# yurimjeon1892/EFGH

Measured on AMD Instinct MI355X. Metric: frame-pairs/sec EFGHNet fwd+bwd (384x1280 RGB + 64x2048 range), whole job, higher is better.
Workload: dtype f32; 1 GPU; BASELINE.json configs[2]: EFGHNet fwd+bwd with efghloss + gradient all-reduce + fused Adam, synthetic 384x1280 RGB + 131072-point sweep, batch=8 per GPU, random-init weights; global_batch=8, points=131072, parallelism=dp1

## Files before the change

### efgh_amd/csrc/wgrad.hip

```cpp
#include "common.h"

namespace {

typedef float f32x16 __attribute__((ext_vector_type(16)));
constexpr int TK = 128, TM = 32, LD = 128;

struct WArgs {
    const float *A; int64_t lda;
    int C, T, K;
    unsigned magicC;
    int Hin, Win, Hv, Wv, sh, sw;
    unsigned long long dhpack, dwpack;
    int Ho, Wo, osh, osw, oh0, ow0;
    const int *table;
    const float *G; int64_t ldg;
    int N;
    int tld;
    long long M; int mchunk;
    float *dW;
    long long zstride;
    unsigned kt, nt;
    long long bsA, bsG, bsD;
};

// ... 64 lines not shown
    }
    float4 rg[NGQ], ra[4];
    auto load_step = [&](long long ms) {
        if (TN != 128) {
#pragma unroll
            for (int q = 0; q < NGQ; ++q) {
                long long m = ms + gr0 + GRS * q;
                float4 g = make_float4(0.f, 0.f, 0.f, 0.f);
                if (m < mend && nin) g = *reinterpret_cast<const float4 *>(MODE == 1 ? git[q].g : p.G + m * p.ldg + n0 + gc4);
                rg[q] = g;
                if (MODE == 1) advance(git[q], n0 + gc4);
            }
        }
#pragma unroll
        for (int q = 0; q < 4; ++q) {
            long long m = ms + r0 + 8 * q;
            float4 g = make_float4(0.f, 0.f, 0.f, 0.f), a = g;
            if (m < mend) {
                if (MODE == 1) {
                    if (TN == 128 && nin) g = *reinterpret_cast<const float4 *>(rit[q].g);
                    if (kin && rit[q].rowok && (unsigned)(rit[q].j * p.sw + dw) < (unsigned)p.Win)
                        a = *reinterpret_cast<const float4 *>(rit[q].a);
                } else {
                    long long arow = -1;
                    if (MODE == 0) arow = m;
                    else if (kin) arow = p.table[m * (MODE == 4 ? p.tld : 16) + t];
                    if (TN == 128 && nin) g = *reinterpret_cast<const float4 *>(p.G + m * p.ldg + n0 + c4);
                    if (kin && arow >= 0) a = *reinterpret_cast<const float4 *>(p.A + arow * p.lda + c);
                }
            }
            if (TN == 128) rg[q] = g;
            ra[q] = a;
            if (MODE == 1) advance(rit[q], n0 + c4);
        }
    };

    f32x16 acc[2][TJ];
#pragma unroll
    for (int i = 0; i < 2; ++i)
#pragma unroll
        for (int j = 0; j < TJ; ++j)
#pragma unroll
            for (int r = 0; r < 16; ++r) acc[i][j][r] = 0.f;

    load_step(mbeg);
    for (long long ms = mbeg; ms < mend; ms += TM) {
#pragma unroll
        for (int q = 0; q < 4; ++q)
            *reinterpret_cast<float4 *>(&As[(r0 + 8 * q) * LD + c4]) = ra[q];
#pragma unroll
        for (int q = 0; q < NGQ; ++q)
            *reinterpret_cast<float4 *>(&Gs[(gr0 + GRS * q) * TN + gc4]) = rg[q];
        __syncthreads();
        if (ms + TM < mend) load_step(ms + TM);
#pragma unroll
        for (int mm = 0; mm < TM / 2; ++mm) {
            float g[2], a[TJ];
#pragma unroll
            for (int i = 0; i < 2; ++i) g[i] = Gs[(mm * 2 + lh) * TN + (wn * 2 + i) * 32 + l31];
#pragma unroll
            for (int j = 0; j < TJ; ++j) a[j] = As[(mm * 2 + lh) * LD + (wk * TJ + j) * 32 + l31];
#pragma unroll
            for (int i = 0; i < 2; ++i)
#pragma unroll
                for (int j = 0; j < TJ; ++j)
                    acc[i][j] = __builtin_amdgcn_mfma_f32_32x32x2f32(g[i], a[j], acc[i][j], 0, 0, 0);
        }
        __syncthreads();
    }
#pragma unroll
    for (int i = 0; i < 2; ++i)
#pragma unroll
        for (int j = 0; j < TJ; ++j) {
            const int k = k0 + (wk * TJ + j) * 32 + l31;
            if (k >= p.K) continue;
#pragma unroll
            for (int r = 0; r < 16; ++r) {
                const int n = n0 + (wn * 2 + i) * 32 + (r & 3) + 8 * (r >> 2) + 4 * lh;
                if (n < p.N) p.dW[(long long)n * p.K + k] = acc[i][j][r];
            }
        }
}

typedef efgh_wgrad_out_desc FoldUnpackArgs;

template <bool UNPACK>
__global__ void __launch_bounds__(256) k_fold_splits(const float4 *part, int zs, long long total4, float4 *dst, const FoldUnpackArgs u) {
    __shared__ float4 red[256];
    const int e = threadIdx.x & 15, zl = threadIdx.x >> 4;
    const long long i = (long long)blockIdx.x * 16 + e;
    float4 a = make_float4(0.f, 0.f, 0.f, 0.f), b = a;
    if (i < total4) {
        int z = zl;
        for (; z + 16 < zs; z += 32) {
            const float4 u = part[(long long)z * total4 + i], v = part[(long long)(z + 16) * total4 + i];
            a.x += u.x; a.y += u.y; a.z += u.z; a.w += u.w;
            b.x += v.x; b.y += v.y; b.z += v.z; b.w += v.w;
        }
        if (z < zs) { const float4 u = part[(long long)z * total4 + i]; a.x += u.x; a.y += u.y; a.z += u.z; a.w += u.w; }
        a.x += b.x; a.y += b.y; a.z += b.z; a.w += b.w;
    }
    red[threadIdx.x] = a;
    __syncthreads();
    for (int h = 8; h; h >>= 1) {
        if (zl < h) {
            const float4 o = red[threadIdx.x + h * 16];
            float4 m = red[threadIdx.x];
            m.x += o.x; m.y += o.y; m.z += o.z; m.w += o.w;
            red[threadIdx.x] = m;
        }
        __syncthreads();
    }
    if (zl == 0 && i < total4) {
        if (!UNPACK) { dst[i] = red[e]; return; }
        const float4 v4 = red[e];
        const float v[4] = {v4.x, v4.y, v4.z, v4.w};
        const long long idx = 4 * i;
        const int c0 = (int)(idx % u.Cp); const long long r = idx / u.Cp;
        const int t = (int)(r % u.T), n = (int)(r / u.T);
        if (n >= u.N) return;
        int ti = 0;
#pragma unroll
        for (int q = 0; q < 16; ++q) if (q == t) ti = u.taps[q];
#pragma unroll
        for (int q = 0; q < 4; ++q) {
            if (c0 + q >= u.C) continue;
            float *d = &u.W[n * u.sn + (c0 + q) * u.sc + ti * u.st];
            *d = u.accumulate ? *d + v[q] : v[q];
        }
    }
}

__global__ void k_unpack_weight(const float *__restrict__ Wp, float *__restrict__ W, int N, int T, int C,
                                int Cp, long long sn, long long sc, long long st, const int4 taps0,
                                const int4 taps1, const int4 taps2, const int4 taps3, int accumulate) {
    const int tp[16] = {taps0.x, taps0.y, taps0.z, taps0.w, taps1.x, taps1.y, taps1.z, taps1.w,
                        taps2.x, taps2.y, taps2.z, taps2.w, taps3.x, taps3.y, taps3.z, taps3.w};
    long long total = (long long)N * T * C;
    for (long long i = (long long)blockIdx.x * blockDim.x + threadIdx.x; i < total;
         i += (long long)gridDim.x * blockDim.x) {
        int c = (int)(i % C); long long r = i / C;
        int t = (int)(r % T); int n = (int)(r / T);
        int ti = 0;
#pragma unroll
        for (int q = 0; q < 16; ++q) if (q == t) ti = tp[q];
        float v = Wp[((long long)n * T + t) * Cp + c];
        float *dst = &W[n * sn + c * sc + ti * st];
        *dst = accumulate ? *dst + v : v;
    }
}

__global__ void __launch_bounds__(256)
k_table_scatter_add(const float *__restrict__ src, const int *__restrict__ table, long long M, int T, int C,
                    float *__restrict__ dst) {
    const int c4n = C >> 2;
    long long total = M * T * c4n;
    for (long long i = (long long)blockIdx.x * 256 + threadIdx.x; i < total; i += (long long)gridDim.x * 256) {
        int cq = (int)(i % c4n); long long r = i / c4n;
        int t = (int)(r % T); long long m = r / T;
        int row = table[m * 16 + t];
        if (row < 0) continue;
        float4 v = *reinterpret_cast<const float4 *>(src + (m * T + t) * C + cq * 4);
        float *d = dst + (long long)row * C + cq * 4;
        atomicAdd(d + 0, v.x); atomicAdd(d + 1, v.y); atomicAdd(d + 2, v.z); atomicAdd(d + 3, v.w);
    }
}

}

bool efgh_launch_fold_splits(const float *part, int zs, long long total, float *dst, hipStream_t st, const efgh_wgrad_out_desc *out) {
    const long long total4 = total / 4;
    const unsigned grid = (unsigned)((total4 + 15) / 16);
    if (out && out->W && out->T >= 1 && out->T <= 16 && out->Cp >= out->C && out->Cp % 4 == 0) {
        const long long row = (long long)out->T * out->Cp;
        if (total % row == 0 && total / row >= out->N && total / row < out->N + 4) {
            k_fold_splits<true><<<grid, 256, 0, st>>>((const float4 *)part, zs, total4, (float4 *)dst, *out);
            return true;
        }
    }
    FoldUnpackArgs none = {};
    k_fold_splits<false><<<grid, 256, 0, st>>>((const float4 *)part, zs, total4, (float4 *)dst, none);
    return false;
}

static int gather_wgrad_impl(const efgh_gemm_desc *d, const float *G, int64_t ldg, float *dWp, float *workspace, int nbatch,
                             int64_t bsG, int64_t bsD, const efgh_wgrad_out_desc *out, void *stream_, int tld = 0);


static long long wgrad_chunks(const efgh_gemm_desc *d, int nbatch, long long *chunk_out) {
    const int K = d->T * d->C;
    const int TN = d->N <= 64 ? 64 : 128;
    const long long kt = (K + TK - 1) / TK, nt = (d->N + TN - 1) / TN;
    static const int occ128[3] = {efgh_wg_per_cu((const void *)k_gather_wgrad<0, 128>, 256, 0), efgh_wg_per_cu((const void *)k_gather_wgrad<1, 128>, 256, 0),
                                  efgh_wg_per_cu((const void *)k_gather_wgrad<2, 128>, 256, 0)};
    static const int occ64[3] = {efgh_wg_per_cu((const void *)k_gather_wgrad<0, 64>, 256, 0), efgh_wg_per_cu((const void *)k_gather_wgrad<1, 64>, 256, 0),
                                 efgh_wg_per_cu((const void *)k_gather_wgrad<2, 64>, 256, 0)};
    const int mode = d->mode >= 0 && d->mode <= 2 ? d->mode : 0;
    return efgh_round_chunks(d->M, kt * nt * nbatch, TN == 128 ? occ128[mode] : occ64[mode], TM, 256, (double)nbatch * d->N * K, chunk_out);
}

extern "C" int64_t efgh_gather_wgrad_workspace(const efgh_gemm_desc *d) {
    if (!d || d->C <= 0 || d->T < 1 || d->N < 1 || d->M < 1) return 0;
    const int nbatch = d->nbatch > 1 ? d->nbatch : 1;
    const long long zs = wgrad_chunks(d, nbatch, nullptr);
    return zs > 1 ? zs * nbatch * (int64_t)d->N * d->T * d->C : 0;
}

extern "C" int efgh_gather_wgrad(const efgh_gemm_desc *d, const float *G, int64_t ldg, float *dWp, float *workspace,
                                 const efgh_wgrad_out_desc *out, void *stream_) {
    return gather_wgrad_impl(d, G, ldg, dWp, workspace, 1, 0, 0, out, stream_);
}

extern "C" int efgh_gather_wgrad_batched(const efgh_gemm_desc *d, const float *G, int64_t ldg, int64_t batch_stride_g,
                                         float *dWp, int64_t batch_stride_dw, float *workspace, void *stream_) {
    EFGH_CHECK_ARG(d && d->mode == 0 && d->nbatch >= 1 && d->nbatch <= 65535);
    EFGH_CHECK_ARG(d->batch_stride_a % 4 == 0 && batch_stride_g % 4 == 0 && batch_stride_dw == (int64_t)d->N * d->C);
    return gather_wgrad_impl(d, G, ldg, dWp, workspace, d->nbatch, batch_stride_g, batch_stride_dw, nullptr, stream_);
}

static int gather_wgrad_impl(const efgh_gemm_desc *d, const float *G, int64_t ldg, float *dWp, float *workspace, int nbatch,
                             int64_t bsG, int64_t bsD, const efgh_wgrad_out_desc *out, void *stream_, int tld) {
    hipStream_t st = (hipStream_t)stream_;
    EFGH_CHECK_ARG(d && d->A && G && dWp);
    EFGH_CHECK_ARG(d->C > 0 && d->C % 4 == 0 && d->T >= 1 && (d->T <= 16 || tld > 0) && d->N >= 1 && d->M >= 1);
    EFGH_CHECK_ARG(tld == 0 || (d->mode == 2 && d->table != nullptr && tld >= d->T && nbatch == 1 && !out));
    EFGH_CHECK_ARG(d->lda % 4 == 0 && ldg % 4 == 0 && d->N % 4 == 0);
    EFGH_CHECK_ARG((((uintptr_t)d->A) & 15) == 0 && (((uintptr_t)G) & 15) == 0 && (((uintptr_t)dWp) & 15) == 0);
    EFGH_CHECK_ARG((int64_t)d->T * d->C < 65536 && d->mode >= 0 && d->mode <= 2);
    WArgs a;
    a.A = d->A; a.lda = d->lda; a.C = d->C; a.T = d->T; a.K = d->T * d->C;
    a.magicC = (unsigned)((0x100000000ULL + d->C - 1) / d->C);
    a.Hin = d->Hin; a.Win = d->Win; a.Hv = d->Hv; a.Wv = d->Wv; a.sh = d->sh; a.sw = d->sw;
    a.dhpack = 0; a.dwpack = 0;
    for (int t = 0; t < 16; ++t) {
        int dh = t < d->T ? d->dh[t] : 0, dw = t < d->T ? d->dw[t] : 0;
        a.dhpack |= (unsigned long long)((dh + 8) & 15) << (4 * t);
        a.dwpack |= (unsigned long long)((dw + 8) & 15) << (4 * t);
    }
    a.Ho = d->Ho; a.Wo = d->Wo; a.osh = d->osh; a.osw = d->osw; a.oh0 = d->oh0; a.ow0 = d->ow0;
    a.table = d->table; a.G = G; a.ldg = ldg; a.N = d->N; a.M = d->M;
    a.bsA = nbatch > 1 ? d->batch_stride_a : 0; a.bsG = bsG; a.bsD = bsD; a.tld = tld;
    if (d->mode == 1) EFGH_CHECK_ARG(d->M == (int64_t)d->B * d->Hv * d->Wv && d->osh >= 1 && d->osw >= 1);
    if (d->mode == 2) EFGH_CHECK_ARG(d->table != nullptr);
    const int TN = a.N <= 64 ? 64 : 128;
    const int kt = (a.K + TK - 1) / TK, nt = (a.N + TN - 1) / TN;
    long long chunk = 0;
    const long long zs = wgrad_chunks(d, nbatch, &chunk);
    a.mchunk = (int)chunk;
    EFGH_CHECK_ARG(zs * kt * nt < 0x7fffffffLL);
    a.kt = (unsigned)kt; a.nt = (unsigned)nt;
    const long long plane = (long long)nbatch * a.N * a.K;
    EFGH_CHECK_ARG(zs == 1 || (workspace && (((uintptr_t)workspace) & 15) == 0));
    a.dW = zs > 1 ? workspace : dWp;
    a.zstride = zs > 1 ? plane : 0;
    const dim3 grid((unsigned)(zs * kt * nt), (unsigned)nbatch);
    if (tld > 0) {
        if (TN == 128) k_gather_wgrad<4, 128><<<grid, 256, 0, st>>>(a);
        else k_gather_wgrad<4, 64><<<grid, 256, 0, st>>>(a);
    } else if (TN == 128) {
        if (d->mode == 0) k_gather_wgrad<0, 128><<<grid, 256, 0, st>>>(a);
        else if (d->mode == 1) k_gather_wgrad<1, 128><<<grid, 256, 0, st>>>(a);
        else k_gather_wgrad<2, 128><<<grid, 256, 0, st>>>(a);
    } else {
        if (d->mode == 0) k_gather_wgrad<0, 64><<<grid, 256, 0, st>>>(a);
        else if (d->mode == 1) k_gather_wgrad<1, 64><<<grid, 256, 0, st>>>(a);
        else k_gather_wgrad<2, 64><<<grid, 256, 0, st>>>(a);
    }
    bool wrote = false;
    if (zs > 1) wrote = efgh_launch_fold_splits(workspace, (int)zs, plane, dWp, st, nbatch == 1 ? out : nullptr);
    EFGH_CHECK_LAUNCH();
    return wrote ? EFGH_WROTE_OUT : EFGH_OK;
}

extern "C" int efgh_blur_r_wgrad(const efgh_gemm_desc *d, int32_t ld, const float *G, int64_t ldg, float *dWp, float *workspace,
                                 void *stream_) {
    EFGH_CHECK_ARG(ld > 0);
    const int rc = gather_wgrad_impl(d, G, ldg, dWp, workspace, 1, 0, 0, nullptr, stream_, ld);
    return rc == EFGH_WROTE_OUT ? EFGH_OK : rc;
}

extern "C" int efgh_unpack_weight(const float *Wp, float *W, int32_t N, int32_t T, int32_t C, int32_t Cp,
                                  int64_t sn, int64_t sc, int64_t stt, const int32_t *tapidx, int32_t accumulate,
                                  void *stream_) {
    EFGH_CHECK_ARG(Wp && W && N > 0 && T > 0 && T <= 16 && C > 0 && Cp >= C);
    int tp[16];
    for (int t = 0; t < 16; ++t) tp[t] = (tapidx && t < T) ? tapidx[t] : (t < T ? t : 0);
    long long total = (long long)N * T * C;
    int grid = (int)((total + 255) / 256);
    if (grid > 8192) grid = 8192;
    k_unpack_weight<<<grid, 256, 0, (hipStream_t)stream_>>>(Wp, W, N, T, C, Cp, sn, sc, stt,
                                                           make_int4(tp[0], tp[1], tp[2], tp[3]),
                                                           make_int4(tp[4], tp[5], tp[6], tp[7]),
                                                           make_int4(tp[8], tp[9], tp[10], tp[11]),
                                                           make_int4(tp[12], tp[13], tp[14], tp[15]), accumulate);
    EFGH_CHECK_LAUNCH();
    return EFGH_OK;
}

extern "C" int efgh_table_scatter_add(const float *src, const int32_t *table, int64_t M, int32_t T, int32_t C,
                                      float *dst, void *stream_) {
    EFGH_CHECK_ARG(src && table && dst && M > 0 && T > 0 && T <= 16 && C % 4 == 0);
    long long total = M * T * (C / 4);
    long long g = (total + 255) / 256;
    k_table_scatter_add<<<(int)(g > 16384 ? 16384 : g), 256, 0, (hipStream_t)stream_>>>(src, table, M, T, C, dst);
    EFGH_CHECK_LAUNCH();
    return EFGH_OK;
}

extern "C" int efgh_debug_occupancy(char *out, int32_t cap) {
    EFGH_CHECK_ARG(out && cap > 64);
    snprintf(out, cap, "k_gather_wgrad<0,128> %d  <1,128> %d  <2,128> %d  <0,64> %d  <1,64> %d  <2,64> %d workgroups per CU",
             efgh_wg_per_cu((const void *)k_gather_wgrad<0, 128>, 256, 0), efgh_wg_per_cu((const void *)k_gather_wgrad<1, 128>, 256, 0),
             efgh_wg_per_cu((const void *)k_gather_wgrad<2, 128>, 256, 0), efgh_wg_per_cu((const void *)k_gather_wgrad<0, 64>, 256, 0),
             efgh_wg_per_cu((const void *)k_gather_wgrad<1, 64>, 256, 0), efgh_wg_per_cu((const void *)k_gather_wgrad<2, 64>, 256, 0));
    return EFGH_OK;
}
```

### efgh_amd/ops.py

```python
import ctypes
import os as _os
import threading
import weakref

import torch

from . import _C
from ._C import c_float, ptr

ACT_NONE, ACT_RELU, ACT_LEAKY = 0, 1, 2


def _L():
    return _C.lib()


def _st():
    return _C.stream_ptr()


def ceil4(n):
    return (n + 3) // 4 * 4


# ... 530 lines not shown
    def regroup():
        return Wp.view(N, S, Ts * C).permute(1, 0, 2).contiguous()
    Wg = _cached(Wp, ('ksplit', S), _ver(Wp), regroup)
    part = _scratch(S * M * N, dev)
    gather_gemm(A, lda, C, Ts, Wg, N, M, part, N, mode=2, table=table, a_off=a_off, batch=(S, 0, N * Ts * C, M * N, Ts),
                flops=flops if flops is not None else 2.0 * M * N * 15 * C, alias_mask=alias_mask)
    b = None
    if bias is not None:
        b = bias if bias.numel() == N else None
        assert b is not None
    _C.check(_L().efgh_fold_planes(ptr(part), S, M, N, ptr(b), act, slope, out.data_ptr() + 4 * out_off, ldo, _st()))


def gather_gemm(A, lda, C, T, Wp, N, M, out, ldo, mode=0, geom=None, table=None, bias=None, scale=None,
                shift=None, residual=None, ldr=0, act=ACT_NONE, slope=0.0, stats=None, a_off=0, out_off=0,
                res_off=0, M_dev=None, flops=None, batch=None, alias_mask=False, bn_bwd=None, pool=False, lazy=None, pre_v=None,
                keep_v=None):
    key = (mode, C, N, T, geom, M, stats is not None, M_dev is not None, batch is not None, pool,
           scale is None and shift is None and residual is None and (bias is None or bias.numel() == N))
    route = gemm_route(*key)
    if (lazy is not None or pre_v is not None) and not (route == 'wino2d' and min(C, N) >= 64):
        raise _C.EfghError('gather_gemm(lazy= / pre_v=) on a launch the 2-D Winograd path does not serve (ask lazy_capable() first)')
    if route == 'blur_r':
        if (geom is not None or batch is not None or M_dev is not None or scale is not None or shift is not None or residual is not None
                or stats is not None or alias_mask or pool or bn_bwd is not None):
            raise _C.EfghError('gather_gemm(mode=MODE_BLUR_R) takes a plain blur launch: bias and activation only')
        blur_r_gemm(A, lda, C, T, Wp, N, M, out, ldo, table, bias=bias, act=act, slope=slope, a_off=a_off, out_off=out_off, flops=flops)
        return None
    if route == 'ksplit':
        return _blur_gemm_ksplit(A, lda, C, Wp, N, M, out, ldo, table, bias, act, slope, a_off, out_off, flops, alias_mask)
    d = _desc(A, lda, C, T, mode, N, M, geom, table, a_off, Wp, out, ldo, out_off, bias, scale, shift, residual, ldr, res_off, act, slope,
              stats, M_dev, batch)
    d.table_alias_mask = 1 if (alias_mask and mode == 2) else 0
    if route == 'sc' and not _sc_aligned(d, lda, ldo, residual, ldr, stats):
        route = gemm_route(*key, aligned=False)
    if pool and route not in ('c4', 'wino2d', 'wino_hpool'):
        raise _C.EfghError('gather_gemm(pool=True) on a launch no pooling epilogue serves (ask pool_fusable() first)')
    ev = _prof_start(PROFILE)
    bn_stats = None
    if route == 'thin':
        if TRACE_THIN is not None:
            TRACE_THIN.append(int(_L().efgh_thin_supported(ctypes.byref(d))))
        _C.check(_L().efgh_thin_gemm(ctypes.byref(d), _st()))
    elif route == 'c4':
        assert lda % 4 == 0
        _C.check((_L().efgh_c4_conv3x3_pooled if pool else _L().efgh_c4_conv3x3)(ctypes.byref(d), _st()))
    elif route == 'sc':
        _C.check(_L().efgh_sc_conv3x3(ctypes.byref(d), _st()))
    elif route == 'wino2d':
        if (bn_bwd is not None and stats is None and BN_BWD_FUSED_2D and out_off == 0 and not pool and bn_bwd.fits(M, N)
                and bn_bwd.y is None and bn_bwd.raw.stride(-2) % 4 == 0):
            rows = _L().efgh_wino2d_stats_rows(geom[0], geom[1], geom[2], N)
            bn_stats = _bn_bwd_sums(d, bn_bwd, rows, N, out.device)
        _wino2d_forward(d, A, a_off, lda, C, N, geom, Wp, pool=pool, lazy=lazy, pre_v=pre_v, keep_v=keep_v)
    elif route == 'wino_hpool':
        _C.check(_L().efgh_wino_conv3x3_hpool(ctypes.byref(d), ptr(wino_weight(Wp, N, C)), _st()))
    elif route == 'wino':
        if bn_bwd is not None and stats is None and BN_BWD_FUSED and out_off == 0 and bn_bwd.fits(M, N):
            rows = _L().efgh_wino_grid_m(geom[0], geom[1], geom[2])
            bn_stats = _bn_bwd_sums(d, bn_bwd, rows, N, out.device)
        _C.check(_L().efgh_wino_conv3x3(ctypes.byref(d), ptr(wino_weight(Wp, N, C)), _st()))
    else:
        _C.check(_L().efgh_gather_gemm(ctypes.byref(d), _st()))
    if ev is not None:
        _prof_end(ev, route, (mode, M, N, T, C), float(flops) if flops is not None else 2.0 * M * N * T * C, PROFILE, PROFILE_WINO,
                  batched=batch is not None)
    return bn_stats


def _bn_bwd_sums(d, src, rows, N, device):
    part = torch.empty((rows, 2, N), dtype=torch.float32, device=device)
    d.stats, d.stats_mode = part.data_ptr(), 1
    d.bn_raw, d.bn_ldraw = src.raw.data_ptr(), src.raw.stride(-2)
    if src.y is not None:
        d.bn_y, d.bn_ldy = src.y.data_ptr(), src.y.stride(-2)
    else:
        d.bn_pscale, d.bn_pshift = src.psc.data_ptr(), src.psh.data_ptr()
    d.bn_mean, d.bn_invstd = src.mean.data_ptr(), src.invstd.data_ptr()
    d.bn_act, d.bn_slope = src.act, src.slope
    return part


GEMM_DMA = True


def apply_switches():
    _L().efgh_gather_gemm_set_dma(1 if GEMM_DMA else 0)


PLANE_DMA = True
PLANE_DMA_NBUF = 0
PROFILE_WINO2D = None
PROFILE_WINO2D_GEMM = None
PLANES_SPLIT = None
PLANE_SPLIT_HITS = [0, 0]


def planes_split_active():
    if PLANES_SPLIT is not None:
        return bool(PLANES_SPLIT)
    return torch.backends.cuda.matmul.fp32_precision == 'tf32'


def _planes_split_now():
    m = TLS.planes_split
    return planes_split_active() if m is None else m


def _batched_plain_gemm(A3, W3, out3, rows, C, N):
    g = _desc(A3, 36 * C, C, 1, 0, N, rows, Wp=W3, out=out3, ldo=36 * N, batch=(36, C, N * C, N))
    ev = _prof_start(PROFILE_WINO2D_GEMM)
    if PLANE_DMA and _L().efgh_plane_gemm_supported(ctypes.byref(g)):
        if _planes_split_now():
            PLANE_SPLIT_HITS[0] += 1
            _C.check(_L().efgh_plane_gemm_x6(ctypes.byref(g), PLANE_DMA_NBUF, _st()))
        else:
            _C.check(_L().efgh_plane_gemm(ctypes.byref(g), PLANE_DMA_NBUF, _st()))
    else:
        _C.check(_L().efgh_gather_gemm(ctypes.byref(g), _st()))
    _prof_end(ev, 'planes', (0, rows, N, 36, C), 2.0 * 36 * rows * C * N, PROFILE_WINO2D_GEMM)


W2V_KEEP = True


POOL_FUSED = True
POOL_HALF = True


def pool_fusable(mode, C, N, geom, residual=None, stats=None):
    if not (POOL_FUSED and residual is None and stats is None and geom is not None and geom[1] >= 2 and geom[2] >= 2):
        return False
    route = gemm_route(mode, C, N, len(geom[7]), geom, geom[0] * geom[3] * geom[4], pool='h')
    if route == 'c4':
        return geom[5] == 1 and geom[6] == 1
    if route == 'wino2d':
        return True
    return 'h' if (route == 'wino_hpool' and POOL_HALF) else False


class LazyAct:
    __slots__ = ('scale', 'shift', 'act', 'slope')

    def __init__(self, scale, shift, act, slope):
        self.scale, self.shift, self.act, self.slope = scale, shift, act, slope


LAZY_ACT = True
W2_BWD_FUSED = True
W2_BWD_FUSED_POOL = True
LAZY_HITS = [0, 0]


def lazy_capable(mode, C, N, geom):
    return geom is not None and min(C, N) >= 64 and gemm_route(mode, C, N, len(geom[7]), geom, 0) == 'wino2d'


def wino2d_input(A, a_off, lda, C, B, H, W, V, lazy=None):
    if lazy is None:
        _C.check(_L().efgh_wino2d_input(A.data_ptr() + 4 * a_off, lda, C, B, H, W, ptr(V), _st()))
    else:
        LAZY_HITS[0] += 1
        _C.check(_L().efgh_wino2d_input_act(A.data_ptr() + 4 * a_off, lda, C, B, H, W, ptr(lazy.scale), ptr(lazy.shift), lazy.act,
                                            lazy.slope, ptr(V), _st()))


def wino2d_bwd_transforms(dy, lddy, raw, ldraw, ybits, psc, psh, mean, invstd, coef, m1, m2, N, B, H, W, act, slope, want_dres):
    T2 = _L().efgh_wino2d_tiles(B, H, W)
    dev = raw.device
    Vd = torch.empty((T2, 36, N), dtype=torch.float32, device=dev)
# ... 972 lines not shown
```

### include/efgh_hip.h

```cpp
#ifndef EFGH_HIP_H
#define EFGH_HIP_H
#include <stdint.h>

#ifdef __cplusplus
extern "C" {
#endif

#define EFGH_OK 0
#define EFGH_E_INVALID (-1)
#define EFGH_E_LAUNCH (-2)
#define EFGH_WROTE_OUT 1

const char *efgh_last_error(void);

#define EFGH_ABI_VERSION 4
int efgh_version(void);

#define EFGH_LATTICE_INFO_H 0
#define EFGH_LATTICE_INFO_ERR 1
#define EFGH_LATTICE_INFO_ALIAS 2
#define EFGH_LATTICE_INFO_CURSOR 3
#define EFGH_LATTICE_INFO_SEG 4
#define EFGH_LATTICE_MAX_SAMPLES 1024

// ... 269 lines not shown
    float bc2_sqrt;
    int32_t skip;
    int32_t nseg;
} efgh_guard_state;
int64_t efgh_grad_guard_workspace(int64_t n);
int efgh_grad_guard_measure(const float *g, int64_t n, const int64_t *bounds, int32_t nseg, double max_norm, float grad_scale,
                            int32_t skip_nonfinite, float beta1, float beta2, int32_t step, void *workspace,
                            efgh_guard_state *state, int32_t grid, void *stream);
int efgh_adam_step_guarded(float *w, const float *g, float *m, float *v, int64_t n, float lr, float beta1, float beta2,
                           float eps, float weight_decay, const efgh_guard_state *state, void *stream);

#define EFGH_ADAM_MAX_GROUPS 16
#define EFGH_ADAM_MAX_SEGMENTS 4096
typedef struct efgh_adam_groups {
    int32_t n_groups;
    int32_t step;
    float beta1, beta2, eps;
    float grad_scale;
    float lr[EFGH_ADAM_MAX_GROUPS];
    float weight_decay[EFGH_ADAM_MAX_GROUPS];
    float decay[EFGH_ADAM_MAX_GROUPS];
    int32_t decoupled[EFGH_ADAM_MAX_GROUPS];
} efgh_adam_groups;
int efgh_adam_step_groups(float *w, const float *g, float *m, float *v, int64_t n, const int64_t *seg_ends,
                          const uint8_t *seg_group, int32_t nseg, const int64_t *host_ends, const uint8_t *host_group,
                          const efgh_adam_groups *groups, const efgh_guard_state *state , int32_t grid,
                          void *stream);

int efgh_grad_drain(float *acc, float *g, int64_t n, int32_t first, void *stream);
int efgh_gimg_valid_count(const float *gdep4, const uint8_t *img_mask, int32_t B, int64_t HW, int64_t *count, void *stream);

typedef struct efgh_txn_state {
    int64_t forward_nonfinite;
    int64_t rolled_back;
    int64_t vetoed_total;
    int32_t first_bad;
    int32_t vetoed;
} efgh_txn_state;
int efgh_txn_snapshot(const float *live_f, float *shadow_f, int64_t nf, const int64_t *live_c, int64_t *shadow_c, int64_t nc,
                      efgh_txn_state *txn, void *stream);
int efgh_txn_probe(const float *live_f, const float *shadow_f, int64_t nf, const int64_t *starts, int32_t nseg, const float *losses,
                   int32_t k, int64_t loss_stride, efgh_txn_state *txn, void *stream);
int efgh_txn_resolve(float *live_f, const float *shadow_f, int64_t nf, int64_t *live_c, const int64_t *shadow_c, int64_t nc,
                     efgh_guard_state *guard, efgh_txn_state *txn, float beta1, float beta2, void *stream);

int efgh_ema_update(float *ema, const float *w, int64_t n, float decay, int32_t warmup, int64_t step,
                    const efgh_guard_state *state , void *stream);
int efgh_ema_swap(float *a, float *b, int64_t n, void *stream);

int efgh_thin_supported(const efgh_gemm_desc *d);
int efgh_thin_gemm(const efgh_gemm_desc *d, void *stream);
int64_t efgh_thin_wgrad_workspace(const efgh_gemm_desc *d);
int efgh_thin_wgrad(const efgh_gemm_desc *d, const float *G, int64_t ldg, float *dWp, float *workspace,
                    const efgh_wgrad_out_desc *out, void *stream);
int efgh_c4n4_supported(const efgh_gemm_desc *d);
int64_t efgh_c4n4_wgrad_workspace(const efgh_gemm_desc *d);
int efgh_c4n4_wgrad(const efgh_gemm_desc *d, const float *G, int64_t ldg, float *dWp, float *workspace,
                    const efgh_wgrad_out_desc *out, void *stream);

int efgh_sc_supported(const efgh_gemm_desc *d);
int32_t efgh_sc_stats_rows(int32_t B, int32_t H, int32_t W);
int efgh_sc_conv3x3(const efgh_gemm_desc *d, void *stream);
int efgh_sc_wgrad_supported(const efgh_gemm_desc *d);
int64_t efgh_sc_wgrad_workspace(const efgh_gemm_desc *d);
int efgh_sc_wgrad(const efgh_gemm_desc *d, const float *G, int64_t ldg, float *dWp, float *workspace,
                  const efgh_wgrad_out_desc *out, void *stream);
int efgh_c4_supported(const efgh_gemm_desc *d);
int32_t efgh_c4_stats_rows(int32_t B, int32_t Ho, int32_t Wo);
int efgh_c4_conv3x3(const efgh_gemm_desc *d, void *stream);
int efgh_c4_pooled_supported(const efgh_gemm_desc *d);
int efgh_c4_conv3x3_pooled(const efgh_gemm_desc *d, void *stream);
int efgh_c4_conv3x3_stats(const efgh_gemm_desc *d, void *stream);
int efgh_c4_conv3x3_pooled_train(const efgh_gemm_desc *d, const float *mean, const float *invstd, float *raw_win, void *stream);
int efgh_c4_pool_bwd_draw(const efgh_gemm_desc *d, const float *dy_pool, const float *mean, const float *invstd, const float *coef,
                          const double *m1, const double *m2, float *draw, void *stream);
int efgh_c4_wgrad_supported(const efgh_gemm_desc *d);
int64_t efgh_c4_wgrad_workspace(const efgh_gemm_desc *d);
int efgh_c4_wgrad(const efgh_gemm_desc *d, const float *G, int64_t ldg, float *dWp, float *workspace,
                  const efgh_wgrad_out_desc *out, void *stream);

int efgh_debug_occupancy(char *out, int32_t cap);

int efgh_gather_gemm_set_dma(int32_t on);

int efgh_plane_gemm_supported(const efgh_gemm_desc *d);
int efgh_plane_gemm(const efgh_gemm_desc *d, int32_t nbuf, void *stream);
int efgh_plane_wgrad_supported(const efgh_gemm_desc *d, int64_t ldg);
int64_t efgh_plane_wgrad_workspace(const efgh_gemm_desc *d);
int efgh_plane_wgrad_batched(const efgh_gemm_desc *d, const float *G, int64_t ldg, int64_t batch_stride_g, float *dWp,
                             int64_t batch_stride_dw, float *workspace, int32_t nbuf, void *stream);

int efgh_plane_gemm_x6(const efgh_gemm_desc *d, int32_t nbuf, void *stream);
int efgh_plane_wgrad_x6_batched(const efgh_gemm_desc *d, const float *G, int64_t ldg, int64_t batch_stride_g, float *dWp,
                                int64_t batch_stride_dw, float *workspace, int32_t nbuf, void *stream);

int efgh_convt_col2im(const float *Y, int64_t ldy, int32_t B, int32_t Hin, int32_t Win, int32_t Ho, int32_t Wo,
                      int32_t O, int32_t pad, const float *scale, const float *shift, int32_t act, float slope,
                      float *out, int64_t ldo, void *stream);
int efgh_convt_im2col(const float *G, int64_t ldg, int32_t B, int32_t Hin, int32_t Win, int32_t Ho, int32_t Wo,
                      int32_t O, int32_t pad, float *Ycol, int64_t ldy, void *stream);

int efgh_corr_pack_cam(const float *cam, const float *cam_mm, int32_t B, int32_t h, int32_t wc, int32_t segw,
                       int32_t nseg, int32_t nsplit, float *Wc, void *stream);
int efgh_corr_fold(const float *P, int32_t B, int32_t nsplit, int64_t Mv, int32_t ldp, int32_t nseg, int32_t segw,
                   int32_t nj, float *logit, float *score, void *stream);
int efgh_norm_bwd(const float *x, const float *dxn, const float *mm, int32_t B, int64_t n, float *part, float *dx, void *stream);
int efgh_corr_planes(const float *x, const float *mm, int32_t B, int32_t h, int32_t w, int32_t w_in_pitch, int32_t wP,
                     float *out, void *stream);
int efgh_corr_unplanes(const float *in, int32_t B, int32_t h, int32_t w, int32_t wP, float *out, void *stream);
int efgh_corr_toeplitz(const float *dl, int32_t B, int32_t nj, int32_t rows, int32_t cols, int32_t colsP, int32_t transpose,
                       float *T, void *stream);

int efgh_wino_supported(const efgh_gemm_desc *d);
int32_t efgh_wino_grid_m(int32_t B, int32_t H, int32_t W);
int efgh_wino_pack(const float *Wp, float *U, int32_t N, int32_t C, void *stream);
int efgh_wino_conv3x3_hpool(const efgh_gemm_desc *d, const float *U, void *stream);
int efgh_wino_conv3x3(const efgh_gemm_desc *d, const float *U, void *stream);
int efgh_wino_wgrad_supported(const efgh_gemm_desc *d);
int64_t efgh_wino_wgrad_workspace(const efgh_gemm_desc *d);
int efgh_wino_wgrad(const efgh_gemm_desc *d, const float *G, int64_t ldg, float *S, float *dWp, const efgh_wgrad_out_desc *out,
                    void *stream);

int efgh_prep_affine_nearest_u8(const uint8_t *in, int32_t h, int32_t w, const int64_t *coef6_host, uint8_t *out,
                                int32_t nh, int32_t nw, void *stream);
int efgh_prep_crop_pad_u8(const uint8_t *in, int32_t h, int32_t w, int32_t oy, int32_t ox, uint8_t *out, int32_t th,
                          int32_t tw, void *stream);
int efgh_prep_resample_u8(const uint8_t *in, int32_t h, int32_t w, int32_t axis, int32_t out_size, const int32_t *bounds,
                          const int32_t *coeffs, int32_t ksize, uint8_t *out, void *stream);
int efgh_prep_hwc_to_chw_u8(const uint8_t *in, int32_t h, int32_t w, uint8_t *chw, uint8_t *mask, void *stream);
int efgh_prep_u8_to_f32_chw_pad(const uint8_t *in, int32_t h, int32_t w, int32_t oy, int32_t ox, float *out, int32_t th,
                                int32_t tw, void *stream);
int32_t efgh_prep_filter_blocks(int32_t n);
int efgh_prep_radius_filter(const float *pcd, const int32_t *pre_idx, int32_t n, int32_t flip_xy, float radius,
                            int32_t *block_scratch, int32_t *keep_idx, int32_t *count, void *stream);
int efgh_prep_gather_transform(const float *pcd, const int32_t *keep_idx, const int32_t *sel, int32_t n_sel,
                               int32_t flip_xy, const double *T34, int32_t num_points, float *out32, double *out64,
                               void *stream);
int efgh_prep_sweeps_filter(const float *pts, int32_t stride, const int32_t *sweep_off, const double *M34,
                            const int32_t *identity, int32_t K, int32_t n_total, const int32_t *pre_idx, int32_t n,
                            int32_t flip_xy, double radius, float ego_x_half, float ego_y_half, int32_t *block_scratch,
                            int32_t *keep_idx, int32_t *count, void *stream);
int efgh_prep_sweeps_gather_transform(const float *pts, int32_t stride, const int32_t *sweep_off, const double *M34,
                                      const int32_t *identity, int32_t K, int32_t n_total, const int32_t *keep_idx,
                                      int32_t n_keep, const int32_t *sel, int32_t n_sel, int32_t flip_xy, const double *T34,
                                      int32_t num_points, float *out32, double *out64, void *stream);
int efgh_prep_sweeps_materialize(const float *pts, int32_t stride, const int32_t *sweep_off, const double *M34,
                                 const int32_t *identity, int32_t K, int32_t n_total, const int32_t *keep_idx, int32_t n,
                                 double *out, void *stream);
int64_t efgh_prep_voxel_workspace(int32_t n);
int efgh_prep_voxel_keep(const float *pts, int32_t stride, int32_t n_rows, const int32_t *keep_in, int32_t n_cap,
                         const int32_t *n_dev, double voxel, void *workspace, int32_t *keep_out, int32_t *count, void *stream);
int efgh_prep_sweeps_voxel_keep(const float *pts, int32_t stride, const int32_t *sweep_off, const double *M34,
                                const int32_t *identity, int32_t K, int32_t n_total, const int32_t *keep_in, int32_t n_cap,
                                const int32_t *n_dev, double voxel, void *workspace, int32_t *keep_out, int32_t *count,
                                void *stream);
#define EFGH_JITTER_MAX_OPS 4
#define EFGH_JITTER_BRIGHTNESS 0
#define EFGH_JITTER_CONTRAST 1
#define EFGH_JITTER_SATURATION 2
#define EFGH_JITTER_HUE 3
int32_t efgh_prep_jitter_partials(int64_t n_pixels);
int efgh_prep_jitter_sum(const uint8_t *in, int64_t n_pixels, const int32_t *ops_host, const float *factors_host, int32_t n_ops,
                         int32_t hue_shift, void *partials, void *stream);
int efgh_prep_jitter_apply(const uint8_t *in, int64_t n_pixels, const int32_t *ops_host, const float *factors_host, int32_t n_ops,
                           int32_t hue_shift, const void *partials, uint8_t *out, void *stream);

// ... 96 lines not shown
```

Baseline: 31.36 frame-pairs/s.

## Add double-buffered direct-to-LDS DMA variant of gather weight-gradient kernel

Adds a new weight-gradient GEMM kernel for gather modes 0 and 1. It loads G and A tiles straight from global memory into a two-slot LDS ring with 16-byte direct-to-LDS copies, so the next tile's load overlaps the MFMA work on the current one. It also remaps block IDs across the XCDs and writes results as float2 stores. The kernel is on by default when the channel count and alignment conditions hold. The cost is a larger dynamic LDS footprint, which may lower occupancy, plus extra index bookkeeping for mode 1.

```diff
diff --git a/efgh_amd/csrc/wgrad.hip b/efgh_amd/csrc/wgrad.hip
--- a/efgh_amd/csrc/wgrad.hip
+++ b/efgh_amd/csrc/wgrad.hip
@@ -170,6 +170,167 @@
         }
 }
 
+__device__ __attribute__((aligned(512))) float g_wgrad_zero[128];
+
+template <int MODE, int TN>
+__global__ void __launch_bounds__(256, 2)
+k_gather_wgrad_dma(const WArgs p0) {
+    extern __shared__ __attribute__((aligned(1024))) float ring[];
+    constexpr int SLOT = TM * (TN + TK);
+    constexpr int TJ = TN == 128 ? 2 : 1;
+    constexpr int NGP = TN == 128 ? 4 : 2;
+    constexpr int GPR = TN == 128 ? 2 : 4;
+    WArgs p = p0;
+    p.A += (long long)blockIdx.y * p0.bsA; p.G += (long long)blockIdx.y * p0.bsG; p.dW += (long long)blockIdx.y * p0.bsD;
+    const int tid = threadIdx.x, lane = tid & 63, wave = __builtin_amdgcn_readfirstlane(tid >> 6);
+    const int wn = TN == 128 ? (wave >> 1) : 0, wk = TN == 128 ? (wave & 1) : wave;
+    const int l31 = lane & 31, lh = lane >> 5;
+    const unsigned ring_lds = lds_addr(ring);
+    const unsigned nblk = gridDim.x, q8 = nblk >> 3, r8 = nblk & 7, xcd = blockIdx.x & 7, within = blockIdx.x >> 3;
+    const unsigned lin = (xcd < r8 ? xcd * (q8 + 1) : r8 * (q8 + 1) + (xcd - r8) * q8) + within;
+    const unsigned per_z = p.kt * p.nt, bz = lin / per_z, rem = lin - bz * per_z;
+    const unsigned by = rem / p.kt, bx = rem - by * p.kt;
+    const int k0 = bx * TK, n0 = by * TN;
+    const long long mbeg = (long long)bz * p.mchunk;
+    long long mend = mbeg + p.mchunk;
+    if (mend > p.M) mend = p.M;
+    if (mbeg >= mend) return;
+    p.dW += (long long)bz * p.zstride;
+
+    const int arow = wave * 8 + lh, grow = wave * 8 + lane / (TN / 4);
+    const int kk = k0 + l31 * 4;
+    const bool kin = kk < p.K;
+    const int t = (int)(((unsigned long long)kk * p.magicC) >> 32);
+    const int c = kk - t * p.C;
+    const int dh = (int)((p.dhpack >> (4 * (t & 15))) & 15) - 8, dw = (int)((p.dwpack >> (4 * (t & 15))) & 15) - 8;
+    const int gcol = n0 + (lane % (TN / 4)) * 4;
+    const bool nin = gcol < p.N;
+    const float *zsrc = g_wgrad_zero + l31 * 4;
+
+    struct RowIt { int j, i; long long b; const float *g, *a; bool rowok; };
+    auto point = [&](RowIt &it) {
+        const long long orow = (it.b * p.Ho + (it.i * p.osh + p.oh0)) * p.Wo + (it.j * p.osw + p.ow0);
+        it.g = p.G + orow * p.ldg + gcol;
+        const int ih = it.i * p.sh + dh;
+        it.rowok = (unsigned)ih < (unsigned)p.Hin;
+        it.a = p.A + ((it.b * p.Hin + ih) * p.Win + (it.j * p.sw + dw)) * p.lda + c;
+    };
+    auto place = [&](RowIt &it, long long m) {
+        it.j = (int)(m % p.Wv); const long long r = m / p.Wv;
+        it.i = (int)(r % p.Hv); it.b = r / p.Hv;
+        point(it);
+    };
+    const long long gstep = (long long)TM * p.osw * p.ldg, astep = (long long)TM * p.sw * p.lda;
+    const bool narrow = p.Wv < 4 * TM;
+    auto advance = [&](RowIt &it) {
+        it.j += TM; it.g += gstep; it.a += astep;
+        if (narrow || it.j >= p.Wv) {
+            while (it.j >= p.Wv) { it.j -= p.Wv; ++it.i; }
+            while (it.i >= p.Hv) { it.i -= p.Hv; ++it.b; }
+            point(it);
+        }
+    };
+    RowIt rit[4], git[NGP];
+    if (MODE == 1) {
+#pragma unroll
+        for (int q = 0; q < 4; ++q) place(rit[q], mbeg + arow + 2 * q);
+        if (TN != 128) {
+#pragma unroll
+            for (int q = 0; q < NGP; ++q) place(git[q], mbeg + grow + GPR * q);
+        }
+    }
+    auto issue = [&](long long ms, int buf) {
+        const unsigned base = ring_lds + (unsigned)(buf * SLOT) * 4u;
+#pragma unroll
+        for (int q = 0; q < NGP; ++q) {
+            const long long m = ms + grow + GPR * q;
+            const float *src = MODE == 1 ? (TN == 128 ? rit[q].g : git[q].g) : p.G + m * p.ldg + gcol;
+            dma16(m < mend && nin ? src : zsrc, base + (unsigned)(wave * NGP + q) * 1024u);
+            if (MODE == 1 && TN != 128) advance(git[q]);
+        }
+#pragma unroll
+        for (int q = 0; q < 4; ++q) {
+            const long long m = ms + arow + 2 * q;
+            bool ok = m < mend && kin;
+            const float *src = p.A + m * p.lda + c;
+            if (MODE == 1) {
+                ok = ok && rit[q].rowok && (unsigned)(rit[q].j * p.sw + dw) < (unsigned)p.Win;
+                src = rit[q].a;
+            }
+            dma16(ok ? src : zsrc, base + (unsigned)(TM * TN) * 4u + (unsigned)(wave * 4 + q) * 1024u);
+            if (MODE == 1) advance(rit[q]);
+        }
+    };
+
+    f32x16 acc[2][TJ];
+#pragma unroll
+    for (int i = 0; i < 2; ++i)
+#pragma unroll
+        for (int j = 0; j < TJ; ++j)
+#pragma unroll
+            for (int r = 0; r < 16; ++r) acc[i][j][r] = 0.f;
+
+    const int nst = (int)((mend - mbeg + TM - 1) / TM);
+    issue(mbeg, 0);
+    const int gx = lh * TN + wn * 64 + 2 * l31, ax = TM * TN + lh * LD + (TN == 128 ? wk * 64 + 2 * l31 : wk * 32 + l31);
+    for (int s = 0; s < nst; ++s) {
+        wait_vm<0>();
+        __builtin_amdgcn_s_barrier();
+        asm volatile("" ::: "memory");
+        if (s + 1 < nst) issue(mbeg + (long long)(s + 1) * TM, (s + 1) & 1);
+        const float *S = ring + (s & 1) * SLOT;
+        if constexpr (TN == 128) {
+            float2 g[2], a[2];
+            g[0] = *reinterpret_cast<const float2 *>(S + gx);
+            a[0] = *reinterpret_cast<const float2 *>(S + ax);
+#pragma unroll
+            for (int mm = 0; mm < TM / 2; ++mm) {
+                if (mm + 1 < TM / 2) {
+                    g[(mm + 1) & 1] = *reinterpret_cast<const float2 *>(S + (mm + 1) * 2 * TN + gx);
+                    a[(mm + 1) & 1] = *reinterpret_cast<const float2 *>(S + (mm + 1) * 2 * LD + ax);
+                }
+                __builtin_amdgcn_sched_barrier(0);
+                const float2 cg = g[mm & 1], ca = a[mm & 1];
+                acc[0][0] = __builtin_amdgcn_mfma_f32_32x32x2f32(cg.x, ca.x, acc[0][0], 0, 0, 0);
+                acc[0][1] = __builtin_amdgcn_mfma_f32_32x32x2f32(cg.x, ca.y, acc[0][1], 0, 0, 0);
+                acc[1][0] = __builtin_amdgcn_mfma_f32_32x32x2f32(cg.y, ca.x, acc[1][0], 0, 0, 0);
+                acc[1][1] = __builtin_amdgcn_mfma_f32_32x32x2f32(cg.y, ca.y, acc[1][1], 0, 0, 0);
+                __builtin_amdgcn_sched_barrier(0);
+            }
+        } else {
+            float2 g[2]; float a[2];
+            g[0] = *reinterpret_cast<const float2 *>(S + gx);
+            a[0] = S[ax];
+#pragma unroll
+            for (int mm = 0; mm < TM / 2; ++mm) {
+                if (mm + 1 < TM / 2) {
+                    g[(mm + 1) & 1] = *reinterpret_cast<const float2 *>(S + (mm + 1) * 2 * TN + gx);
+                    a[(mm + 1) & 1] = S[(mm + 1) * 2 * LD + ax];
+                }
+                __builtin_amdgcn_sched_barrier(0);
+                const float2 cg = g[mm & 1]; const float ca = a[mm & 1];
+                acc[0][0] = __builtin_amdgcn_mfma_f32_32x32x2f32(cg.x, ca, acc[0][0], 0, 0, 0);
+                acc[1][0] = __builtin_amdgcn_mfma_f32_32x32x2f32(cg.y, ca, acc[1][0], 0, 0, 0);
+                __builtin_amdgcn_sched_barrier(0);
+            }
+        }
+    }
+#pragma unroll
+    for (int q = 0; q < 2; ++q)
+#pragma unroll
+        for (int r = 0; r < 16; ++r) {
+            const int n = n0 + wn * 64 + 2 * ((r & 3) + 8 * (r >> 2) + 4 * lh) + q;
+            if (n >= p.N) continue;
+            if constexpr (TN == 128) {
+                const int k = k0 + wk * 64 + 2 * l31;
+                if (k < p.K) *reinterpret_cast<float2 *>(p.dW + (long long)n * p.K + k) = make_float2(acc[q][0][r], acc[q][1][r]);
+            } else {
+                const int k = k0 + wk * 32 + l31;
+                if (k < p.K) p.dW[(long long)n * p.K + k] = acc[q][0][r];
+            }
+        }
+}
+
 typedef efgh_wgrad_out_desc FoldUnpackArgs;
 
 template <bool UNPACK>
@@ -274,8 +435,29 @@
 static int gather_wgrad_impl(const efgh_gemm_desc *d, const float *G, int64_t ldg, float *dWp, float *workspace, int nbatch,
                              int64_t bsG, int64_t bsD, const efgh_wgrad_out_desc *out, void *stream_, int tld = 0);
 
-
-static long long wgrad_chunks(const efgh_gemm_desc *d, int nbatch, long long *chunk_out) {
+static int g_wgrad_dma = 1;
+static std::atomic<unsigned long long> g_wgrad_dma_raised[4];
+
+static bool wgrad_dma_ok(const efgh_gemm_desc *d) {
+    return g_wgrad_dma != 0 && (d->mode == 0 || d->mode == 1) && d->C % 32 == 0 && !d->M_dev && d->lda % 4 == 0
+           && (((uintptr_t)d->A) & 15) == 0;
+}
+
+template <int MODE, int TN>
+static size_t wgrad_dma_lds() { return (size_t)2 * TM * (TN + TK) * sizeof(float); }
+
+template <int MODE, int TN>
+static int launch_wgrad_dma(const WArgs &a, dim3 grid, hipStream_t st) {
+    const size_t lds = wgrad_dma_lds<MODE, TN>();
+    if (!efgh_raise_lds_once(g_wgrad_dma_raised[MODE * 2 + (TN == 128)], (const void *)k_gather_wgrad_dma<MODE, TN>, (int)lds)) {
+        efgh_set_error("%s:%d: cannot raise the dynamic LDS limit of k_gather_wgrad_dma", __FILE__, __LINE__);
+        return EFGH_E_LAUNCH;
+    }
+    k_gather_wgrad_dma<MODE, TN><<<grid, 256, lds, st>>>(a);
+    return EFGH_OK;
+}
+
+static long long wgrad_chunks(const efgh_gemm_desc *d, int nbatch, bool dma, long long *chunk_out) {
     const int K = d->T * d->C;
     const int TN = d->N <= 64 ? 64 : 128;
     const long long kt = (K + TK - 1) / TK, nt = (d->N + TN - 1) / TN;
@@ -283,14 +465,19 @@
                                   efgh_wg_per_cu((const void *)k_gather_wgrad<2, 128>, 256, 0)};
     static const int occ64[3] = {efgh_wg_per_cu((const void *)k_gather_wgrad<0, 64>, 256, 0), efgh_wg_per_cu((const void *)k_gather_wgrad<1, 64>, 256, 0),
                                  efgh_wg_per_cu((const void *)k_gather_wgrad<2, 64>, 256, 0)};
+    static const int dma128[2] = {efgh_wg_per_cu((const void *)k_gather_wgrad_dma<0, 128>, 256, wgrad_dma_lds<0, 128>()),
+                                  efgh_wg_per_cu((const void *)k_gather_wgrad_dma<1, 128>, 256, wgrad_dma_lds<1, 128>())};
+    static const int dma64[2] = {efgh_wg_per_cu((const void *)k_gather_wgrad_dma<0, 64>, 256, wgrad_dma_lds<0, 64>()),
+                                 efgh_wg_per_cu((const void *)k_gather_wgrad_dma<1, 64>, 256, wgrad_dma_lds<1, 64>())};
     const int mode = d->mode >= 0 && d->mode <= 2 ? d->mode : 0;
-    return efgh_round_chunks(d->M, kt * nt * nbatch, TN == 128 ? occ128[mode] : occ64[mode], TM, 256, (double)nbatch * d->N * K, chunk_out);
+    const int occ = dma && g_wgrad_dma == 2 ? (TN == 128 ? dma128[mode] : dma64[mode]) : (TN == 128 ? occ128[mode] : occ64[mode]);
+    return efgh_round_chunks(d->M, kt * nt * nbatch, occ, TM, 256, (double)nbatch * d->N * K, chunk_out);
 }
 
 extern "C" int64_t efgh_gather_wgrad_workspace(const efgh_gemm_desc *d) {
     if (!d || d->C <= 0 || d->T < 1 || d->N < 1 || d->M < 1) return 0;
     const int nbatch = d->nbatch > 1 ? d->nbatch : 1;
-    const long long zs = wgrad_chunks(d, nbatch, nullptr);
+    const long long zs = wgrad_chunks(d, nbatch, wgrad_dma_ok(d), nullptr);
     return zs > 1 ? zs * nbatch * (int64_t)d->N * d->T * d->C : 0;
 }
 
@@ -333,7 +520,8 @@
     const int TN = a.N <= 64 ? 64 : 128;
     const int kt = (a.K + TK - 1) / TK, nt = (a.N + TN - 1) / TN;
     long long chunk = 0;
-    const long long zs = wgrad_chunks(d, nbatch, &chunk);
+    const bool dma = tld == 0 && wgrad_dma_ok(d);
+    const long long zs = wgrad_chunks(d, nbatch, dma, &chunk);
     a.mchunk = (int)chunk;
     EFGH_CHECK_ARG(zs * kt * nt < 0x7fffffffLL);
     a.kt = (unsigned)kt; a.nt = (unsigned)nt;
@@ -342,7 +530,12 @@
     a.dW = zs > 1 ? workspace : dWp;
     a.zstride = zs > 1 ? plane : 0;
     const dim3 grid((unsigned)(zs * kt * nt), (unsigned)nbatch);
-    if (tld > 0) {
+    if (dma) {
+        int rc;
+        if (TN == 128) rc = d->mode == 0 ? launch_wgrad_dma<0, 128>(a, grid, st) : launch_wgrad_dma<1, 128>(a, grid, st);
+        else rc = d->mode == 0 ? launch_wgrad_dma<0, 64>(a, grid, st) : launch_wgrad_dma<1, 64>(a, grid, st);
+        if (rc != EFGH_OK) return rc;
+    } else if (tld > 0) {
         if (TN == 128) k_gather_wgrad<4, 128><<<grid, 256, 0, st>>>(a);
         else k_gather_wgrad<4, 64><<<grid, 256, 0, st>>>(a);
     } else if (TN == 128) {
@@ -358,6 +551,12 @@
     if (zs > 1) wrote = efgh_launch_fold_splits(workspace, (int)zs, plane, dWp, st, nbatch == 1 ? out : nullptr);
     EFGH_CHECK_LAUNCH();
     return wrote ? EFGH_WROTE_OUT : EFGH_OK;
+}
+
+extern "C" int efgh_gather_wgrad_set_dma(int32_t on) {
+    const int old = g_wgrad_dma;
+    g_wgrad_dma = on == 2 ? 2 : (on != 0);
+    return old;
 }
 
 extern "C" int efgh_blur_r_wgrad(const efgh_gemm_desc *d, int32_t ld, const float *G, int64_t ldg, float *dWp, float *workspace,
@@ -397,9 +596,14 @@
 
 extern "C" int efgh_debug_occupancy(char *out, int32_t cap) {
     EFGH_CHECK_ARG(out && cap > 64);
-    snprintf(out, cap, "k_gather_wgrad<0,128> %d  <1,128> %d  <2,128> %d  <0,64> %d  <1,64> %d  <2,64> %d workgroups per CU",
+    snprintf(out, cap, "k_gather_wgrad<0,128> %d  <1,128> %d  <2,128> %d  <0,64> %d  <1,64> %d  <2,64> %d  "
+             "k_gather_wgrad_dma<0,128> %d  <1,128> %d  <0,64> %d  <1,64> %d workgroups per CU",
              efgh_wg_per_cu((const void *)k_gather_wgrad<0, 128>, 256, 0), efgh_wg_per_cu((const void *)k_gather_wgrad<1, 128>, 256, 0),
              efgh_wg_per_cu((const void *)k_gather_wgrad<2, 128>, 256, 0), efgh_wg_per_cu((const void *)k_gather_wgrad<0, 64>, 256, 0),
-             efgh_wg_per_cu((const void *)k_gather_wgrad<1, 64>, 256, 0), efgh_wg_per_cu((const void *)k_gather_wgrad<2, 64>, 256, 0));
+             efgh_wg_per_cu((const void *)k_gather_wgrad<1, 64>, 256, 0), efgh_wg_per_cu((const void *)k_gather_wgrad<2, 64>, 256, 0),
+             efgh_wg_per_cu((const void *)k_gather_wgrad_dma<0, 128>, 256, wgrad_dma_lds<0, 128>()),
+             efgh_wg_per_cu((const void *)k_gather_wgrad_dma<1, 128>, 256, wgrad_dma_lds<1, 128>()),
+             efgh_wg_per_cu((const void *)k_gather_wgrad_dma<0, 64>, 256, wgrad_dma_lds<0, 64>()),
+             efgh_wg_per_cu((const void *)k_gather_wgrad_dma<1, 64>, 256, wgrad_dma_lds<1, 64>()));
     return EFGH_OK;
 }
diff --git a/efgh_amd/ops.py b/efgh_amd/ops.py
--- a/efgh_amd/ops.py
+++ b/efgh_amd/ops.py
@@ -636,10 +636,12 @@
 
 
 GEMM_DMA = True
+WGRAD_DMA = True
 
 
 def apply_switches():
     _L().efgh_gather_gemm_set_dma(1 if GEMM_DMA else 0)
+    _L().efgh_gather_wgrad_set_dma(int(WGRAD_DMA))
 
 
 PLANE_DMA = True
diff --git a/include/efgh_hip.h b/include/efgh_hip.h
--- a/include/efgh_hip.h
+++ b/include/efgh_hip.h
@@ -375,6 +375,7 @@
 int efgh_debug_occupancy(char *out, int32_t cap);
 
 int efgh_gather_gemm_set_dma(int32_t on);
+int efgh_gather_wgrad_set_dma(int32_t on);
 
 int efgh_plane_gemm_supported(const efgh_gemm_desc *d);
 int efgh_plane_gemm(const efgh_gemm_desc *d, int32_t nbuf, void *stream);
```

Measured after the change: 31.62 frame-pairs/s, median of 6. Within noise of the previous version (+0.8%).
